# NikolaZubic/2dimageto3dmodel

Measured on NVIDIA H100. Metric: render+loss+GAN images/sec (cfg3: cfg2 render+loss at batch 32 + conv-GAN 256x256 G/D iteration, 1 G : 2 D, Adam), higher is better.
Workload: dtype tf32 (convs) / f32

## Files before the change

### 2dimageto3dmodel_b200/b3d/__init__.py

```python
import ctypes
import os

import torch

_HERE = os.path.dirname(os.path.abspath(__file__))
LIB_PATH = os.path.join(_HERE, "libb3d.so")

MODE_REFERENCE = 0
MODE_PAPER = 1
_MODES = {"R": MODE_REFERENCE, "reference": MODE_REFERENCE, "P": MODE_PAPER, "paper": MODE_PAPER,
          0: MODE_REFERENCE, 1: MODE_PAPER}


class B3DError(RuntimeError):
    pass


def _load():
    if not os.path.exists(LIB_PATH):
        raise B3DError(f"{LIB_PATH} is missing: build it with `make` (or __graft_entry__.build()). "
                       "There is no CPU fallback.")
    lib = ctypes.CDLL(LIB_PATH)
    lib.b3d_last_error.restype = ctypes.c_char_p
    lib.b3d_last_variant.restype = ctypes.c_char_p
# ... 6 lines not shown

_vp = ctypes.c_void_p
_i = ctypes.c_int
_f = ctypes.c_float
_sz = ctypes.c_size_t
_ll = ctypes.c_longlong


_signed = []


def _sig(name, *argtypes):
    fn = getattr(lib, name)
    fn.argtypes = list(argtypes)
    fn.restype = ctypes.c_int
    _signed.append(name)
    return fn


_sig("b3d_pc_bin_count", _i)
_sig("b3d_inception_input", _vp, _i, _i, _i, _i, _i, _i, _i, _vp, _vp)
_sig("b3d_maxpool3x3s2_nhwc", _vp, _i, _i, _i, _i, _vp, _i, _vp)
_sig("b3d_mean_hw_nhwc", _vp, _i, _i, _i, _vp, _vp)
_sig("b3d_fid_accumulate", _vp, _i, _i, _vp, _vp, _vp)
_sig("b3d_pc_project", _vp, _vp, _i, _i, _i, _f, _f, _vp, _vp, _vp, _vp, _vp, _vp, _vp)
_sig("b3d_pc_silhouette_fwd_hosttaps", _vp, _vp, _vp, _i, _vp, _i, _i, _i, _i, _vp, _vp, _sz, _vp)
_sig("b3d_pc_silhouette_bwd_hosttaps", _vp, _vp, _vp, _i, _vp, _vp, _i, _i, _i, _i, _vp, _vp, _vp, _sz, _vp)
_sig("b3d_pc_project_bwd", _vp, _vp, _vp, _vp, _i, _i, _i, _f, _f, _vp, _vp, _vp)
_sig("b3d_pc_splat_grid", _vp, _i, _i, _i, _i, _vp, _vp)
_sig("b3d_mesh_face_setup", _vp, _vp, _vp, _i, _vp, _i, _i, _i, _i, _vp, _vp, _vp, _vp)
_sig("b3d_mesh_render_fwd", _vp, _vp, _vp, _vp, _i, _i, _i, _i, _i, _i, _vp, _vp, _vp, _vp, _vp)
_sig("b3d_conv2d_tf32", _vp, _vp, _vp, _vp, _i, _i, _i, _i, _i, _i, _i, _i, _vp, _vp, _i, _i, _i, _i, _i, _i, _i, _i, _i,
     _f, _vp, _i, _vp, _i, _i, _vp, _vp)
_sig("b3d_conv2d_wgrad_tf32", _vp, _vp, _vp, _i, _i, _i, _i, _i, _i, _i, _i, _i, _i, _i, _i, _i, _i, _i, _vp)
_sig("b3d_conv2d_thin_fwd", _vp, _vp, _vp, _vp, _i, _i, _i, _i, _i, _i, _i, _i, _i, _i, _i, _i, _i, _f, _vp)
_sig("b3d_conv2d_thin_wgrad", _vp, _vp, _vp, _i, _i, _i, _i, _i, _i, _i, _i, _i, _i, _i, _i, _vp)
_sig("b3d_vertex_pipeline_fwd", _vp, _ll, _ll, _ll, _ll, _i, _i, _vp, _vp, _i, _i, _vp, _vp, _vp, _vp, _vp, _vp, _vp)
_sig("b3d_vertex_pipeline_bwd", _vp, _vp, _vp, _vp, _vp, _i, _i, _i, _i, _vp, _vp, _vp, _vp, _vp, _vp, _vp, _vp, _vp)
_sig("b3d_bank_forward", _vp, _vp, _i, _vp, _i, _vp, _i, _vp, _sz, _vp, _i, _vp)
_sig("b3d_bank_backward", _vp, _vp, _i, _vp, _i, _vp, _vp, _vp, _vp)
_sig("b3d_up2_fold", _vp, _vp, _i, _i, _vp)
_sig("b3d_pad_x_fwd", _vp, _vp, _ll, _i, _i, _i, _i, _vp)
_sig("b3d_pad_x_bwd", _vp, _vp, _ll, _i, _i, _i, _i, _vp)
_sig("b3d_stem_input_fwd", _vp, _vp, _vp, _i, _i, _i, _i, _i, _i, _i, _vp)
_sig("b3d_stem_input_bwd", _vp, _vp, _i, _i, _i, _i, _i, _i, _i, _vp)
_sig("b3d_leaky_bwd", _vp, _vp, _vp, _ll, _f, _vp)
_sig("b3d_fold_rows_fwd", _vp, _vp, _i, _i, _i, _i, _i, _i, _i, _vp)
_sig("b3d_fold_rows_bwd", _vp, _vp, _i, _i, _i, _i, _i, _i, _i, _vp)
_sig("b3d_wrap_x_inplace", _vp, _ll, _i, _i, _i, _i, _vp)
_sig("b3d_wrap_x_bwd_inplace", _vp, _ll, _i, _i, _i, _i, _vp)
_sig("b3d_pad_leaky_bias_bwd", _vp, _vp, _vp, _vp, _ll, _i, _i, _i, _i, _f, _vp)
_sig("b3d_vox_blur_axis", _vp, _vp, _vp, _i, _i, _i, _i, _i, _vp)
_sig("b3d_vox_scale_clamp", _vp, _vp, _vp, _i, _i, _vp)
_sig("b3d_vox_scale_clamp_bwd", _vp, _vp, _vp, _vp, _vp, _i, _i, _vp)
_sig("b3d_vox_termination", _vp, _i, _i, _i, _vp, _vp, _vp)
_sig("b3d_vox_termination_bwd", _vp, _vp, _i, _i, _i, _vp, _vp)
_sig("b3d_vox_splat_sorted", _vp, _vp, _i, _i, _i, _i, _vp, _vp)
_sig("b3d_vox_clamp01", _vp, ctypes.c_longlong, _vp)
_sig("b3d_vox_gather", _vp, _vp, _vp, _vp, _i, _i, _i, _i, _vp, _vp)
_sig("b3d_cbn_act_fwd", _vp, _vp, _vp, _vp, _i, _i, _vp, _i, _i, _i, _i, _i, _i, _i, _f, _i, _vp)
_sig("b3d_cbn_act_bwd1", _vp, _vp, _vp, _vp, _vp, _i, _i, _vp, _vp, _i, _vp, _vp, _i, _i, _vp, _vp, _i, _i, _i, _i, _i, _i, _i, _i,
     _f, _i, _vp)
_sig("b3d_cbn_act_bwd2", _vp, _vp, _vp, _vp, _vp, _i, _vp, _vp, _i, _f, _i, _i, _i, _i, _vp)
_sig("b3d_bn_sums", _vp, _ll, _i, _vp, _vp)
_sig("b3d_cbn_prepare", _vp, _i, _i, _i, _vp, ctypes.c_double, _f, _f, _i, _vp, _vp, _vp, _vp, _vp, _vp, _vp, _vp, _i, _i, _vp)
_sig("b3d_cbn_bwd_reduce", _vp, _vp, _i, _vp, _vp, _i, _i, _vp)
# ... 119 lines not shown
```

### 2dimageto3dmodel_b200/b3d/conv.py

```python
import ctypes

import torch

from . import B3DError, check, dev, last_variant, lib, ptr, stream_ptr
from .bank import LayerWeights

VARIANT_LOG = None


def _conv_call(fn, *args):
    rc = fn(*args)
    if VARIANT_LOG is not None and rc == 0:
        VARIANT_LOG.extend(v for v in last_variant().split(";") if v)
    return rc


def _ints(v):
    return (ctypes.c_int * len(v))(*v)


def _pad_last(t, mult):
    c = t.shape[-1]
    return t if c % mult == 0 else torch.nn.functional.pad(t, (0, mult - c % mult))


def taps_layout(weight):
    co, ci, kh, kw = weight.shape
    return weight.permute(2, 3, 0, 1).reshape(kh * kw, co, ci).contiguous()


def _d_layout(wf):
    return _pad_last(wf.transpose(1, 2), 32).contiguous()


def _thin(Cout, Cin, kh, kw, stride):
    return Cout <= 4 and Cin % 64 == 0 and kh == 5 and kw == 5 and stride == 1


class _ConvOpts(ctypes.Structure):
    _fields_ = [("mask", ctypes.c_void_p), ("mask_slope", ctypes.c_float), ("stats_sum_only", ctypes.c_int),
                ("x_row_pitch", ctypes.c_int), ("nclass", ctypes.c_int), ("class_ooy", ctypes.c_int * 4), ("class_oox", ctypes.c_int * 4)]


def _fprop(x, wt, bias, kh, kw, pad_y=0, stride=1, leaky=1.0, pad_out=0, pad_mode=1, x_crop=0, stats=None, fold_kh=0,
           fold_pad=0):
    N, H, W, _ = x.shape
    _, Cout, Cin = wt.shape
    if x_crop and stride != 1:
        raise B3DError("conv2d: x_crop needs stride 1")
    if pad_out and Cout % 4:
        raise B3DError("conv2d: pad_out needs Cout % 4 == 0")
    Hout = (H + 2 * fold_pad - fold_kh + 1) if fold_kh else (H + 2 * pad_y - kh) // stride + 1
    Wout = (W - 2 * x_crop - kw) // stride + 1
    OW = Wout + 2 * pad_out
    out = torch.empty(N, Hout, OW, Cout, device=x.device, dtype=torch.float32)
    optr = ctypes.c_void_p(out.data_ptr() + 4 * pad_out * Cout)
    b = dev(bias, "bias") if bias is not None else None
    st = stream_ptr(x)
    if _thin(Cout, Cin, kh, kw, stride):
        check(_conv_call(lib.b3d_conv2d_thin_fwd, ptr(x), ptr(wt), ptr(b), optr, N, H, W, Cin, Hout, Wout, Cout, kh, kw, pad_y,
                         x_crop, OW, Cout, float(leaky), st))
    else:
        if stats is not None and (bias is not None or leaky != 1.0 or stride != 1):
            raise B3DError("conv2d: output statistics are taken before bias / activation (plain stride-1 convs only)")
        dy = [r - pad_y for r in range(kh) for _ in range(kw)]
        dx = [s + x_crop for _ in range(kh) for s in range(kw)]
        check(_conv_call(lib.b3d_conv2d_tf32, ptr(x), ptr(wt), ptr(b), optr, N, H, W, Cin, Hout, Wout, Cout, kh * kw, _ints(dy),
                         _ints(dx), stride, stride, Hout, OW, Cout, 1, 1, 0, 0, float(leaky), None, 0, ptr(stats), fold_kh,
                         fold_pad, None, st))
    if pad_out:
        check(lib.b3d_wrap_x_inplace(ptr(out), N * Hout, Wout, Cout, pad_out, pad_mode, st))
    return out


def stride2_classes(kh, kw, pad_y, H, W):
    out = []
    for cy in range(2):
        for cx in range(2):
            rs = [(r, s) for r in range(kh) for s in range(kw) if (cy + pad_y - r) % 2 == 0 and (cx - s) % 2 == 0]
            out.append((cy, cx, rs, [(cy + pad_y - r) // 2 for r, s in rs], [(cx - s) // 2 for r, s in rs],
                        (H - cy + 1) // 2, (W - cx + 1) // 2))
    return out


def _merge_parity_classes(classes):
    return len(classes) == 4 and all(c[2] for c in classes) and len({(len(c[2]), c[5], c[6]) for c in classes}) == 1


def _dgrad(gy, wd, in_hw, kh, kw, pad_y=0, stride=1, x_crop=0, g_pitch=0, mask=None, slope=1.0, sums=None):
    gy = _pad_last(gy, 32)
    N, Hout, Wout, Cop = gy.shape
    Cin = wd.shape[1]
# ... 158 lines not shown
    x = xp_nchw.permute(0, 2, 3, 1)
    out = _UpConv.apply(x, lw.wf, lw_sc.wf if lw_sc is not None else None, lw, lw_sc, stats)
    y, sc = out if lw_sc is not None else (out, None)
    return y.permute(0, 3, 1, 2), sc.permute(0, 3, 1, 2) if sc is not None else None


def conv2d_nhwc(x, weight, bias=None, pad_y=0, stride=1, leaky=1.0, wt=None, pad_out=0, pad_mode=1, x_crop=0):
    x = dev(x, "x")
    Cout, Cin_w, kh, kw = weight.shape
    if Cin_w != x.shape[3]:
        raise B3DError(f"conv2d: input has {x.shape[3]} channels, weight expects {Cin_w}")
    wt = dev(wt if wt is not None else taps_layout(weight), "weight")
    return _fprop(x, wt, bias, kh, kw, pad_y, stride, leaky, pad_out, pad_mode, x_crop)


def conv2d_dgrad_nhwc(dy_, weight, in_hw, pad_y=0, stride=1, x_crop=0):
    Cout, Cin, kh, kw = weight.shape
    wd = _d_layout(weight.permute(2, 3, 0, 1).reshape(kh * kw, Cout, Cin))
    return _dgrad(dev(dy_, "grad_output"), wd, in_hw, kh, kw, pad_y, stride, x_crop)


def conv2d_wgrad_nhwc(dy_, x, kh, kw, pad_y=0, stride=1, x_crop=0):
    return _wgrad(dev(dy_, "grad_output"), dev(x, "input"), kh, kw, pad_y, stride, x_crop)


class ActLink:
    __slots__ = ("armed", "slope", "pad", "mode", "ptr", "shape", "want_gb", "gb", "done")

    def __init__(self):
        self.armed = self.done = False
        self.gb = None


class _Conv(torch.autograd.Function):
    @staticmethod
    def forward(ctx, x, w, bias, lw, pad_y, stride, leaky, pad_out, pad_mode, x_crop, stats=None, fold_raw=0, link_in=None,
                link_out=None, fold_fwd=False):
        x = dev(x.detach(), "x")
        if lw.wp is not None:
            raise B3DError("conv2d: a layer registered with up2 runs through conv2d_up2_banked")
        Cx = x.shape[3]
        fold_pad = 0
        if fold_raw:
            if not lw.fold or Cx != 8 or lw.Cin != 8 or stride != 1 or x_crop:
                raise B3DError("conv2d: on-the-fly fold needs a folded 8-channel stride-1 stem")
            fold_pad = pad_y
        elif Cx != lw.Cinp:
            if lw.fold or Cx != lw.Cin:
                raise B3DError(f"conv2d: input has {Cx} channels, the layer expects {lw.Cinp if lw.fold else lw.Cin}")
            x = _pad_last(x, 32)
        kh, kw = (1, lw.kw) if lw.fold else (lw.kh, lw.kw)
        if lw.fold:
            pad_y = 0
        wf, b = dev(lw.wf.detach(), "weight"), bias.detach() if bias is not None else None
        if fold_raw and fold_fwd:
            from .ew import fold_rows
            out = _fprop(fold_rows(x, lw.kh, fold_pad, lw.Cinp), wf, b, kh, kw, 0, stride, leaky, pad_out, pad_mode, x_crop, stats)
        else:
            out = _fprop(x, wf, b, kh, kw, pad_y, stride, leaky, pad_out, pad_mode, x_crop, stats, fold_raw, fold_pad)
        ctx.save_for_backward(x, out if (leaky != 1.0 or pad_out) else None)
        ctx.lw = lw
        ctx.cfg = (pad_y, stride, Cx, bias is not None, leaky, pad_out, pad_mode, x_crop, kh, kw, fold_raw, fold_pad)
        thin = _thin(lw.Cout, lw.Cinp, kh, kw, stride)
        ctx.link_in = link_in if (link_in is not None and link_in.armed and link_in.ptr == x.data_ptr() and link_in.shape == tuple(x.shape)
                                  and Cx == lw.Cinp and lw.Cinp % 32 == 0 and not fold_raw and not thin) else None
        ctx.link_out = None
        if link_out is not None and pad_out and leaky != 1.0 and lw.Cout % 32 == 0 and not thin:
            link_out.armed, link_out.slope, link_out.pad, link_out.mode = True, float(leaky), int(pad_out), int(pad_mode)
            link_out.ptr, link_out.shape, link_out.done = out.data_ptr(), tuple(out.shape), False
            link_out.want_gb = bias is not None and bool(ctx.needs_input_grad[2])
            ctx.link_out = link_out
        return out

    @staticmethod
    def backward(ctx, gy):
        x, y = ctx.saved_tensors
        lw = ctx.lw
        pad_y, stride, Cx, has_bias, leaky, pad_out, pad_mode, x_crop, kh, kw, fold_raw, fold_pad = ctx.cfg
        Cout, Cin = lw.Cout, lw.Cinp
        N, H, W, _ = x.shape
        gy = dev(gy, "grad_output")
        st = stream_ptr(gy)
        gb = None
        want_gb = has_bias and ctx.needs_input_grad[2]
        g_pitch = 0
        link_out = ctx.link_out
        if link_out is not None and link_out.done:
            link_out.done = False
# ... 10 lines not shown
            check(lib.b3d_pad_leaky_bias_bwd(ptr(gy), ptr(y), ptr(masked), ptr(gb), N * Ho, OW - 2 * pad_out, Cout, pad_out,
                                             pad_mode, float(leaky), st))
            gy = masked
        elif leaky != 1.0:
            masked = torch.empty_like(gy)
            check(lib.b3d_leaky_bwd(ptr(gy), ptr(y), ptr(masked), gy.numel(), float(leaky), st))
            gy = masked
        if gb is None and want_gb:
            gb = gy.sum(dim=(0, 1, 2))
        gx = gw = None
        if ctx.needs_input_grad[0]:
            link_in = ctx.link_in
            sums = torch.zeros(2 * Cin, device=gy.device, dtype=torch.float64) if link_in is not None and link_in.want_gb else None
            gx = _dgrad(gy, lw.wd if lw.wd is not None else _d_layout(lw.wf.detach()), (gy.shape[1] if fold_raw else H, W), kh,
                        kw, pad_y, stride, x_crop, g_pitch, x if link_in is not None else None,
                        link_in.slope if link_in is not None else 1.0, sums)
            if link_in is not None:
                check(lib.b3d_wrap_x_bwd_inplace(ptr(gx), N * H, W - 2 * link_in.pad, Cin, link_in.pad, link_in.mode, st))
                link_in.gb = sums[:Cin].float() if sums is not None else None
                link_in.done = True
            if fold_raw:
                graw = torch.empty(N, H, W, Cx, device=gy.device, dtype=torch.float32)
                check(lib.b3d_fold_rows_bwd(ptr(gx), ptr(graw), N, H, W, Cx, lw.kh, fold_pad, Cin, st))
                gx = graw
            elif Cx != Cin:
                gx = gx[..., :Cx]
        if ctx.needs_input_grad[1]:
            if fold_raw:
                gw = _wgrad(gy, x, kh, kw, fold_pad, stride, x_crop, lw.df, g_pitch, fold_raw, Cin)
            else:
                gw = _wgrad(gy, x, kh, kw, pad_y, stride, x_crop, lw.df, g_pitch)
            if lw.df is None:
                gw = gw[:, :lw.Cin]
        return gx, gw, gb, None, None, None, None, None, None, None, None, None, None, None, None


def fold_kh_weight(weight, cpad=0):
    Cout, Cin, kh, kw = weight.shape
    w = weight.permute(0, 2, 1, 3).reshape(Cout, kh * Cin, 1, kw)
    return torch.nn.functional.pad(w, (0, 0, 0, 0, 0, cpad)) if cpad else w


def conv2d(x_nchw, weight, bias=None, pad_y=0, stride=1, leaky=1.0, pad_out=0, pad_mode=1, x_crop=0):
    x = x_nchw.permute(0, 2, 3, 1)
    Cout, Cin, kh, kw = weight.shape
    if stride == 1 and kh > 1 and Cin * kh <= 64:
        from .ew import fold_rows
        cpad = (-kh * Cin) % 32
        x = fold_rows(x, kh, pad_y, kh * Cin + cpad)
        weight = fold_kh_weight(weight, cpad)
        Cout, Cin, kh, kw = weight.shape
        pad_y = 0
    lw = LayerWeights(dict(Cout=Cout, Cin=Cin, kh=kh, kw=kw, fold=0, Cinp=-(-Cin // 32) * 32, Coutp=-(-Cout // 32) * 32,
                           Tp=kh * kw))
    lw.wf = _pad_last(taps_layout(weight.detach()), 32)
    y = _Conv.apply(x, weight, bias, lw, int(pad_y), int(stride), float(leaky), int(pad_out), int(pad_mode), int(x_crop))
    return y.permute(0, 3, 1, 2)


def conv2d_banked(x_nchw, lw, pad_y=0, stride=1, leaky=1.0, pad_out=0, pad_mode=1, x_crop=0, stats=None, link_in=None, link_out=None):
    x = x_nchw.permute(0, 2, 3, 1)
    fold_raw, fold_fwd = 0, False
    if lw.fold:
        Wout = x.shape[2] - lw.kw + 1
        if (lw.Cin == 8 and lw.kw == 5 and lw.Cinp == 64 and stride == 1 and not x_crop and Wout % 128 == 0
                and x.shape[0] * x.shape[1] * (Wout // 128) >= 2 * torch.cuda.get_device_properties(x.device).multi_processor_count):
            fold_raw = lw.kh
            fold_fwd = torch.is_grad_enabled() and lw.wf.requires_grad
        else:
            from .ew import fold_rows
            x = fold_rows(x, lw.kh, pad_y, lw.Cinp)
    y = _Conv.apply(x, lw.wf, lw.bias, lw, int(pad_y), int(stride), float(leaky), int(pad_out), int(pad_mode), int(x_crop), stats,
                    fold_raw, link_in, link_out, fold_fwd)
    return y.permute(0, 3, 1, 2)
```

### 2dimageto3dmodel_b200/csrc/b3d_core.cu

```cuda
#include <atomic>
#include <stdarg.h>
#include <string.h>

#include "b3d_common.cuh"

namespace b3d {
static thread_local char g_err[512] = "";
static thread_local char g_variant[256] = "";
static std::atomic<uint64_t> g_launches{0};

void set_error(const char* fmt, ...) {
    va_list ap;
    va_start(ap, fmt);
    vsnprintf(g_err, sizeof(g_err), fmt, ap);
    va_end(ap);
}
void clear_variant() { g_variant[0] = 0; }
void add_variant(const char* fmt, ...) {
    size_t n = strlen(g_variant);
    if (n + 2 >= sizeof(g_variant)) return;
    if (n) g_variant[n++] = ';';
    va_list ap;
    va_start(ap, fmt);
    vsnprintf(g_variant + n, sizeof(g_variant) - n, fmt, ap);
    va_end(ap);
}
void count_launch(int n) { g_launches.fetch_add((uint64_t)n, std::memory_order_relaxed); }
}

extern "C" {
const char* b3d_last_error(void) { return b3d::g_err; }
const char* b3d_last_variant(void) { return b3d::g_variant; }
int b3d_version(void) { return 440; }
uint64_t b3d_launch_count(void) { return b3d::g_launches.load(std::memory_order_relaxed); }
}
```

### 2dimageto3dmodel_b200/csrc/tc_conv.cu

```cuda
#include "tc_common.cuh"

namespace {

constexpr int BM = 128;
constexpr int BK = 32;
constexpr int MMA_K = 8;
constexpr int MAX_TAPS = 25;
constexpr int NTHREADS = 384;

struct ConvParams {
    int N, Hout, Wout, Cout;
    int BW, BH, BI;
    int tiles_x, tiles_y;
    int xbase;
    int ntaps, kslices;
    int sy, sx;
    int dy[MAX_TAPS], dx[MAX_TAPS];
    int wtap[MAX_TAPS];
    int OH, OW, OC, osy, osx;
    float leaky;
    double* stats;
    int fold;
    int fold_y0;
    int mask;
// ... 19 lines not shown

__device__ __forceinline__ uint32_t mask_offset(int px, int ch) { return px * 128 + ((((ch >> 2) ^ px) & 7) << 4) + (ch & 3) * 4; }

template <int BN>
constexpr bool kCoop = BN > 128;
template <int BN>
constexpr int kBlocks = (kCoop<BN> ? BN / 2 : BN) / 64;
template <int BN>
constexpr int kEmptyArrivals = kCoop<BN> ? 8 : 4;
template <int BN>
constexpr int kLeaderArrivals = kEmptyArrivals<BN> / (kCoop<BN> ? 2 : 1);
static_assert(kLeaderArrivals<64> == 4 && kLeaderArrivals<128> == 4 && kLeaderArrivals<256> == 4,
              "a leader stands for the 4 warps of its warpgroup");
template <int BN>
constexpr int kMaskGroup = kCoop<BN> ? 4 : 2;
__host__ __device__ constexpr int mask_chunk_channel(int i, int G) { return 128 * ((i % G) / 2) + 64 * (i / G) + 32 * (i % 2); }

template <int BN, int STAGES, int KW, bool FOLD>
__device__ __forceinline__ void mainloop(float (&acc)[kBlocks<BN>][BM / 2], unsigned char* base, uint64_t* full, uint64_t* empty,
                                         int KI, uint32_t& git, uint32_t& phase, int cb, bool leader, const int* shift) {
    constexpr int A_BYTES = CSmem<BN, STAGES, KW>::A_BYTES, STAGE = CSmem<BN, STAGES, KW>::STAGE_BYTES;
    for (int it = 0; it < KI; ++it, ++git) {
        const int s = git % STAGES;
        tc::mbar_wait(full + s, (phase >> s) & 1);
        phase ^= 1u << s;
        const uint32_t a = tc::smem_u32(base + s * STAGE), b = a + A_BYTES + cb * 128;
        tc::wgmma_fence();
#pragma unroll
        for (int t = 0; t < KW; ++t) {
            const uint32_t shifted = a + (KW > 1 ? shift[t] * 128 : 0);
#pragma unroll
            for (int k = 0; k < BK / MMA_K; ++k) {
                const uint32_t acc_flag = (it | t | k) ? 1u : 0u;
                const uint64_t dp = FOLD ? tc::desc_k32(a + k * (BM * 32)) : tc::desc_k128(shifted + k * MMA_K * 4);
#pragma unroll
                for (int m = 0; m < kBlocks<BN>; ++m)
                    tc::Wgmma<BM>::mma(acc[m], tc::desc_k128(b + t * (BN * 128) + m * (64 * 128) + k * MMA_K * 4), dp, acc_flag);
            }
        }
        tc::wgmma_commit();
        tc::wgmma_wait<1>();
        if (it > 0 && leader) tc::mbar_arrive(empty + (git - 1) % STAGES, kLeaderArrivals<BN>);
    }
    tc::wgmma_wait<0>();
    if (KI > 0 && leader) tc::mbar_arrive(empty + (git - 1) % STAGES, kLeaderArrivals<BN>);
}

struct TileAt {
    int n0, y0, x0;
    size_t base;
    int lbw, lbwh;
};
__device__ __forceinline__ void tile_origin(const ConvParams& p, TileAt& t, int tile, int cls) {
    t.x0 = p.xbase + (tile % p.tiles_x) * p.BW;
    t.y0 = (tile / p.tiles_x) % p.tiles_y * p.BH;
    t.n0 = tile / (p.tiles_x * p.tiles_y) * p.BI;
    t.base = (((size_t)t.n0 * p.OH + (size_t)(p.osy * t.y0 + p.cooy[cls])) * p.OW + (size_t)(p.osx * t.x0 + p.coox[cls])) * p.OC;
}
__device__ __forceinline__ bool tile_pixel(const ConvParams& p, const TileAt& t, int px, uint32_t& rel) {
    const int bi = px >> t.lbwh, by = (px >> t.lbw) & (p.BH - 1), bx = px & (p.BW - 1);
    rel = bi * p.esn + by * p.esy + bx * p.esx;
    return t.n0 + bi < p.N && t.y0 + by < p.Hout && t.x0 + bx < p.Wout;
}

template <int G, int STAGES>
__device__ __forceinline__ void mask_bits(uint32_t (&neg)[2], uint32_t mstage, int cw, int lane, uint64_t* empty, uint32_t g0) {
    int q;
// ... 37 lines not shown
        for (int e1 = 0; e1 < 2; ++e1) {
            uint32_t rel;
            const bool valid = tile_pixel(p, t, 8 * j + q + e1, rel);
#pragma unroll
            for (int e2 = 0; e2 < 2; ++e2) {
                float v = acc[4 * j + 2 * e2 + e1];
                if constexpr (MASKED) v *= (neg[j / 8] >> (4 * (j % 8) + 2 * e2 + e1)) & 1u ? p.mslope : 1.f;
                v = valid ? v : 0.f;
                sum[e2] += v;
                sq[e2] += v * v;
                if (valid && cok[e2]) {
                    const float o = v + bv[e2];
                    out0[rel + 8 * e2] = o >= 0.f ? o : o * p.leaky;
                }
            }
        }
    }
    if (p.stats) {
#pragma unroll
        for (int e = 0; e < 2; ++e) {
            sum[e] += __shfl_xor_sync(0xffffffffu, sum[e], 1);
            sum[e] += __shfl_xor_sync(0xffffffffu, sum[e], 2);
            sq[e] += __shfl_xor_sync(0xffffffffu, sq[e], 1);
            sq[e] += __shfl_xor_sync(0xffffffffu, sq[e], 2);
            if ((lane & 3) == 0 && cok[e]) {
                atomicAdd(p.stats + c0 + cw + 8 * e, (double)sum[e]);
                if (!p.stats_sum) atomicAdd(p.stats + p.Cout + c0 + cw + 8 * e, (double)sq[e]);
            }
        }
    }
}

constexpr int PRODUCER_REGS = 24, CONSUMER_REGS = 240;

template <int BN, int STAGES, int KW>
__global__ void __launch_bounds__(NTHREADS, 1)
conv_wgmma_kernel(const __grid_constant__ CUtensorMap tmap_x, const __grid_constant__ CUtensorMap tmap_w,
                  const __grid_constant__ CUtensorMap tmap_m, const ConvParams p, const float* __restrict__ bias,
                  float* __restrict__ out, int tiles, int work_items) {
    using S = CSmem<BN, STAGES, KW>;
    constexpr bool COOP = kCoop<BN>;
    constexpr int OWNERS = COOP ? 1 : 2;
    constexpr int G = kMaskGroup<BN>;
    static_assert(G <= STAGES, "the mask stages of one block do not fit the ring");
    extern __shared__ unsigned char smem_raw[];
    unsigned char* base = reinterpret_cast<unsigned char*>((reinterpret_cast<uintptr_t>(smem_raw) + 1023) & ~uintptr_t(1023));
    uint64_t* full = reinterpret_cast<uint64_t*>(base + STAGES * S::STAGE_BYTES);
    uint64_t* empty = full + OWNERS * STAGES;
    static_assert((OWNERS + 1) * STAGES * 8 <= 256, "barriers do not fit their area");
    if (threadIdx.x == 0) {
        tc::tma_prefetch_desc(&tmap_x);
        tc::tma_prefetch_desc(&tmap_w);
        if (p.mask) tc::tma_prefetch_desc(&tmap_m);
        for (int s = 0; s < STAGES; ++s) {
            for (int o = 0; o < OWNERS; ++o) tc::mbar_init(full + o * STAGES + s, 1);
            tc::mbar_init(empty + s, kEmptyArrivals<BN>);
        }
        tc::fence_barrier_init();
    }
    __syncthreads();
    const int KI = p.ntaps / KW * p.kslices;
    const int MS = p.mask ? BN / 32 : 0;
    const int wg = threadIdx.x >> 7;

    if (wg == 0) {
        tc::setmaxnreg_dec<PRODUCER_REGS>();
        if (threadIdx.x == 0) {
            uint32_t git = 0;
            for (int w = blockIdx.x, k = 0; w < work_items; w += gridDim.x, ++k) {
                uint64_t* fb = full + (COOP ? 0 : (k & 1) * STAGES);
                const int cls = w % p.ncls, wq = w / p.ncls, tb = cls * p.ntaps;
                int t = wq % tiles;
                const int c0 = (wq / tiles) * BN;
                const int x0 = p.xbase + (t % p.tiles_x) * p.BW;
                t /= p.tiles_x;
                const int y0 = (t % p.tiles_y) * p.BH, n0 = (t / p.tiles_y) * p.BI;
                for (int it = 0; it < KI; ++it, ++git) {
                    const int s = git % STAGES;
                    tc::mbar_wait(empty + s, ((git / STAGES) & 1) ^ 1);
                    const int tap = it / p.kslices * KW, ks = it % p.kslices;
                    unsigned char* a = base + s * S::STAGE_BYTES;
                    tc::mbar_arrive_expect_tx(fb + s, S::TX_BYTES);
                    if (KW > 1)
                        tc::tma_load_4d(a, &tmap_x, fb + s, ks * BK, x0 + p.dx0, y0 + p.dy[tb + tap], n0);
                    else if (p.fold)
                        tc::tma_load_4d(a, &tmap_x, fb + s, 0, x0 + p.dx[tb + tap], y0 + p.fold_y0 + 4 * ks, n0);
                    else
                        tc::tma_load_4d(a, &tmap_x, fb + s, ks * BK, p.sx * x0 + p.dx[tb + tap], p.sy * y0 + p.dy[tb + tap], n0);
                    tc::tma_load_3d(a + S::A_BYTES, &tmap_w, fb + s, ks * BK, c0, p.wtap[tb + tap]);
                }
                const int mx = p.osx * x0 + p.coox[cls], my = p.osy * y0 + p.cooy[cls];
                for (int m = 0; m < MS; ++m, ++git) {
                    const int s = git % STAGES;
                    tc::mbar_wait(empty + s, ((git / STAGES) & 1) ^ 1);
                    tc::mbar_arrive_expect_tx(fb + s, MASK_BYTES);
                    tc::tma_load_4d(base + s * S::STAGE_BYTES, &tmap_m, fb + s, c0 + mask_chunk_channel(m, G), mx, my, n0);
                }
            }
        }
        return;
    }
    tc::setmaxnreg_inc<CONSUMER_REGS>();

    const int h = wg - 1, tid = threadIdx.x & 127, lane = tid & 31;
    float acc[kBlocks<BN>][BM / 2];
#pragma unroll
    for (int m = 0; m < kBlocks<BN>; ++m)
#pragma unroll
        for (int i = 0; i < BM / 2; ++i) acc[m][i] = 0.f;
    uint32_t git = 0, phase = 0;
    const uint32_t ring = tc::smem_u32(base);
    TileAt at;
    at.lbw = __ffs(p.BW) - 1;
    at.lbwh = at.lbw + __ffs(p.BH) - 1;
    uint64_t* fb = full + (COOP ? 0 : h * STAGES);
    const int cb = COOP ? 128 * h : 0;
    const int cw = (tid >> 5) * 16 + (lane >> 2);
    const int mine = (COOP ? 2 * h : 0) + (tid >> 6);
    for (int k = COOP ? 0 : h;; k += COOP ? 1 : 2) {
        const int w = blockIdx.x + k * gridDim.x;
        if (w >= work_items) break;
        git = (uint32_t)k * (KI + MS);
        const int wq = w / p.ncls, tile = wq % tiles, c0 = (wq / tiles) * BN + cb;
        tile_origin(p, at, tile, w % p.ncls);
        if (KW == 1 && p.fold) mainloop<BN, STAGES, KW, true>(acc, base, fb, empty, KI, git, phase, cb, tid == 0, p.shift);
        else mainloop<BN, STAGES, KW, false>(acc, base, fb, empty, KI, git, phase, cb, tid == 0, p.shift);
        uint32_t neg[kBlocks<BN>][2] = {};
        if (p.mask) {
#pragma unroll
            for (int m = 0; m < kBlocks<BN>; ++m, git += G) {
                uint32_t mstage = 0;
#pragma unroll
                for (int i = 0; i < G; ++i) {
                    const int s = (git + i) % STAGES;
                    tc::mbar_wait(fb + s, (phase >> s) & 1);
                    phase ^= 1u << s;
                    if (i == mine) mstage = ring + s * S::STAGE_BYTES;
                }
                mask_bits<G, STAGES>(neg[m], mstage, cw, lane, empty, git);
            }
        }
#pragma unroll
        for (int m = 0; m < kBlocks<BN>; ++m) {
            if (p.mask) epilogue_block<true>(acc[m], neg[m], p, at, bias, out, c0 + 64 * m, cw, lane);
            else epilogue_block<false>(acc[m], neg[m], p, at, bias, out, c0 + 64 * m, cw, lane);
        }
    }
}

struct WgradParams {
    int N, Hout, Wout, Cout, Cin;
    int BWk, BHk;
    int kx, ky;
    int kh, kw, pad_y, st;
    int xoff;
    int splits;
    int tapmajor;
    int tstep;
// ... 371 lines not shown
    }
    return best;
}

template <int BN, int STAGES, int KW = 1>
int launch_conv(const CUtensorMap& mx, const CUtensorMap& mw, const CUtensorMap& mm, const ConvParams& p, const float* bias, float* out,
                int tiles, cudaStream_t st) {
    using S = CSmem<BN, STAGES, KW>;
    static_assert(S::TOTAL <= 227 * 1024, "conv pipeline does not fit shared memory");
    B3D_CUDA_OK(cudaFuncSetAttribute(conv_wgmma_kernel<BN, STAGES, KW>, cudaFuncAttributeMaxDynamicSharedMemorySize, S::TOTAL));
    const int work = tiles * b3d::ceil_div(p.Cout, BN) * p.ncls;
    const int sms = tc::num_sms();
    conv_wgmma_kernel<BN, STAGES, KW><<<work < sms ? work : sms, NTHREADS, S::TOTAL, st>>>(mx, mw, mm, p, bias, out, tiles, work);
    B3D_LAUNCH_OK();
    if (KW > 1) b3d::add_variant("conv_wgmma_rowwin<%d,%d,%d>", BN, KW, STAGES);
    else b3d::add_variant("conv_wgmma<%d,%d>", BN, STAGES);
    return B3D_OK;
}

template <int BN>
int launch_rowwin(int kw, const CUtensorMap& mx, const CUtensorMap& mw, const CUtensorMap& mm, const ConvParams& p, const float* bias,
                  float* out, int tiles, cudaStream_t st) {
    if (kw == 2) return launch_conv<BN, BN == 64 ? 5 : 4, 2>(mx, mw, mm, p, bias, out, tiles, st);
    if (kw == 3) return launch_conv<BN, BN == 64 ? 4 : 3, 3>(mx, mw, mm, p, bias, out, tiles, st);
    return launch_conv<BN, BN == 64 ? 3 : 2, 5>(mx, mw, mm, p, bias, out, tiles, st);
}

int pow2_floor(int v) {
    int p = 1;
    while (p * 2 <= v) p *= 2;
    return p;
}

}

extern "C" {

int b3d_conv2d_tf32(const float* x, const float* wt, const float* bias, float* out, int N, int H, int W, int Cin,
                    int Hout, int Wout, int Cout, int ntaps, const int* dy, const int* dx, int sy, int sx, int OH,
                    int OW, int OC, int osy, int osx, int ooy, int oox, float leaky, const int* wtap,
                    int wtaps_total, double* stats, int fold_kh, int fold_pad, const b3d_conv_opts* opts, void* stream) {
    B3D_REQUIRE(N > 0 && H > 0 && W > 0 && Hout > 0 && Wout > 0 && Cout > 0, B3D_EINVAL, "b3d_conv2d_tf32: bad sizes");
    B3D_REQUIRE(Cin > 0 && Cin % BK == 0, B3D_EINVAL, "b3d_conv2d_tf32: Cin=%d must be a multiple of %d", Cin, BK);
    B3D_REQUIRE(ntaps >= 1 && ntaps <= MAX_TAPS && dy && dx, B3D_EINVAL, "b3d_conv2d_tf32: bad taps");
    B3D_REQUIRE(x && wt && out, B3D_EINVAL, "b3d_conv2d_tf32: null pointer");
    B3D_REQUIRE(sy >= 1 && sy <= 2 && sx >= 1 && sx <= 2, B3D_EINVAL, "b3d_conv2d_tf32: stride must be 1 or 2");
    if (!wtap) wtaps_total = ntaps;
    B3D_REQUIRE(wtaps_total >= ntaps || wtap, B3D_EINVAL, "b3d_conv2d_tf32: bad weight tap count");
    for (int t = 0; wtap && t < ntaps; ++t)
        B3D_REQUIRE(wtap[t] >= 0 && wtap[t] < wtaps_total, B3D_EINVAL, "b3d_conv2d_tf32: weight tap %d out of range", wtap[t]);
    B3D_CHECK_ALIGNED(x);
    B3D_CHECK_ALIGNED(wt);
    b3d::clear_variant();

    const float* mask = opts ? opts->mask : nullptr;
    const float mslope = opts ? opts->mask_slope : 1.f;
    B3D_REQUIRE(!mask || (reinterpret_cast<uintptr_t>(mask) % 16 == 0 && OC % 4 == 0), B3D_EINVAL,
                "b3d_conv2d_tf32: the mask needs a 16-byte aligned base and OC %% 4 == 0 (OC=%d)", OC);
    const int stats_sum = (opts && opts->stats_sum_only) ? 1 : 0;
    const int xpitch = (opts && opts->x_row_pitch) ? opts->x_row_pitch : W;
    const int ncls = (opts && opts->nclass > 1) ? opts->nclass : 1;
    B3D_REQUIRE(ncls <= 4 && ntaps % ncls == 0 && (ncls == 1 || (sy == 1 && sx == 1 && fold_kh == 0)), B3D_EINVAL,
                "b3d_conv2d_tf32: nclass=%d needs <= 4 equal tap groups of a stride-1 launch", ncls);
    const int tpc = ntaps / ncls;
    int cooy[4] = {ooy, ooy, ooy, ooy}, coox[4] = {oox, oox, oox, oox};
    for (int c = 0; c < ncls && ncls > 1; ++c) { cooy[c] = opts->class_ooy[c]; coox[c] = opts->class_oox[c]; }
    B3D_REQUIRE(xpitch >= W && (fold_kh == 0 || xpitch == W), B3D_EINVAL, "b3d_conv2d_tf32: x_row_pitch=%d must be >= W=%d (and absent with the on-the-fly fold)", xpitch, W);
    if (fold_kh > 0) {
        B3D_REQUIRE(fold_kh <= 8 && Cin == 32 * ((8 * fold_kh + 31) / 32) && sy == 1 && sx == 1 && !wtap && Wout % BM == 0,
                    B3D_EINVAL, "b3d_conv2d_tf32: on-the-fly fold needs 8 input channels, stride 1 and Wout %% 128 == 0 (Wout=%d)", Wout);
    }
    bool tiles = ncls == 4 && osy == 2 && osx == 2 && OH == 2 * Hout && OW == 2 * Wout;
    for (int c = 0, seen = 0; tiles && c < 4; ++c) {
        const int bit = 1 << (2 * cooy[c] + coox[c]);
// ... 33 lines not shown
        const int wspan = xhi - xlo;
        ConvParams p{};
        p.N = N; p.Hout = Hout; p.Wout = xhi; p.Cout = Cout; p.xbase = xlo;
        p.BW = pow2_floor(wspan < BM ? wspan : BM);
        p.BH = pow2_floor(Hout < BM / p.BW ? Hout : BM / p.BW);
        p.BI = BM / (p.BW * p.BH);
        p.tiles_x = b3d::ceil_div(wspan, p.BW);
        p.tiles_y = b3d::ceil_div(Hout, p.BH);
        const int tiles = p.tiles_x * p.tiles_y * b3d::ceil_div(N, p.BI);
        p.ntaps = tpc; p.kslices = Cin / BK; p.sy = sy; p.sx = sx; p.ncls = ncls;
        for (int t = 0; t < ntaps; ++t) { p.dy[t] = dy[t]; p.dx[t] = dx[t]; p.wtap[t] = wtap ? wtap[t] : t; }
        for (int c = 0; c < 4; ++c) { p.cooy[c] = cooy[c]; p.coox[c] = coox[c]; }
        p.OH = OH; p.OW = OW; p.OC = OC; p.osy = osy; p.osx = osx;
        p.leaky = leaky;
        p.stats = stats;
        p.mask = mask != nullptr; p.mslope = mslope; p.stats_sum = stats_sum;
        p.fold = fold_kh; p.fold_y0 = -fold_pad;
        {
            const unsigned long long esn = p.BI > 1 ? (unsigned long long)OH * OW * OC : 0, esy = p.BH > 1 ? (unsigned long long)osy * OW * OC : 0,
                                     esx = (unsigned long long)osx * OC;
            B3D_REQUIRE((p.BI - 1) * esn + (p.BH - 1) * esy + (p.BW - 1) * esx + OC < (1ull << 32), B3D_EINVAL,
                        "b3d_conv2d_tf32: a %d x %d x %d pixel tile spans more than 2^32 elements of the output", p.BI, p.BH, p.BW);
            p.esn = (uint32_t)esn; p.esy = (uint32_t)esy; p.esx = (uint32_t)esx;
        }
        CUtensorMap mm{};
        if (mask) {
            const uint64_t dims[4] = {(uint64_t)OC, (uint64_t)OW, (uint64_t)OH, (uint64_t)N};
            const uint64_t strides[3] = {(uint64_t)OC * 4, (uint64_t)OW * OC * 4, (uint64_t)OH * OW * OC * 4};
            const uint32_t box[4] = {(uint32_t)BK, (uint32_t)(osx * (p.BW - 1) + 1), (uint32_t)(osy * (p.BH - 1) + 1), (uint32_t)p.BI};
            const uint32_t es[4] = {1, (uint32_t)osx, (uint32_t)osy, 1};
            if (int rc = tc::make_tmap_f32(&mm, mask, 4, dims, strides, box, es)) return rc;
        }
        CUtensorMap mx;
        if (g_kw && wspan >= BM) {
            p.dx0 = g_step > 0 ? dx[0] : dx[g_kw - 1];
            for (int t = 0; t < g_kw; ++t) p.shift[t] = dx[t] - p.dx0;
            const uint64_t dims[4] = {(uint64_t)Cin, (uint64_t)W, (uint64_t)H, (uint64_t)N};
            const uint64_t strides[3] = {(uint64_t)Cin * 4, (uint64_t)xpitch * Cin * 4, (uint64_t)H * xpitch * Cin * 4};
            const uint32_t box[4] = {(uint32_t)BK, (uint32_t)(BM + g_kw - 1), 1, 1};
            if (int rc = tc::make_tmap_f32(&mx, x, 4, dims, strides, box)) return rc;
            CUtensorMap mwr;
            const uint64_t wdims[3] = {(uint64_t)Cin, (uint64_t)Cout, (uint64_t)wtaps_total};
            const uint64_t wstrides[2] = {(uint64_t)Cin * 4, (uint64_t)Cout * Cin * 4};
            const uint32_t wbox[3] = {(uint32_t)BK, (uint32_t)BN, (uint32_t)((g_kw - 1) * g_wstep + 1)};
            const uint32_t wes[3] = {1, 1, (uint32_t)g_wstep};
            if (int rc = tc::make_tmap_f32(&mwr, wt, 3, wdims, wstrides, wbox, wes)) return rc;
            return BN == 128 ? launch_rowwin<128>(g_kw, mx, mwr, mm, p, bias, out, tiles, st)
                             : launch_rowwin<64>(g_kw, mx, mwr, mm, p, bias, out, tiles, st);
        }
        if (fold_kh > 0) {
            B3D_REQUIRE(p.BH == 1 && p.BI == 1, B3D_EINVAL, "b3d_conv2d_tf32: on-the-fly fold needs one-row tiles");
            const uint64_t dims[4] = {8, (uint64_t)W, (uint64_t)H, (uint64_t)N};
            const uint64_t strides[3] = {32, (uint64_t)W * 32, (uint64_t)H * W * 32};
            const uint32_t box[4] = {8, (uint32_t)p.BW, 4, 1};
            if (int rc = tc::make_tmap_f32(&mx, x, 4, dims, strides, box, nullptr, CU_TENSOR_MAP_SWIZZLE_32B)) return rc;
        } else {
            const uint64_t dims[4] = {(uint64_t)Cin, (uint64_t)W, (uint64_t)H, (uint64_t)N};
            const uint64_t strides[3] = {(uint64_t)Cin * 4, (uint64_t)xpitch * Cin * 4, (uint64_t)H * xpitch * Cin * 4};
            const uint32_t box[4] = {(uint32_t)BK, (uint32_t)(sx * (p.BW - 1) + 1), (uint32_t)(sy * (p.BH - 1) + 1), (uint32_t)p.BI};
            const uint32_t es[4] = {1, (uint32_t)sx, (uint32_t)sy, 1};
            if (int rc = tc::make_tmap_f32(&mx, x, 4, dims, strides, box, es)) return rc;
        }
        if (BN == 256) return launch_conv<256, 4>(mx, mw, mm, p, bias, out, tiles, st);
        if (BN == 128) return launch_conv<128, 6>(mx, mw, mm, p, bias, out, tiles, st);
        return launch_conv<64, 8>(mx, mw, mm, p, bias, out, tiles, st);
    };
    const int bw_full = pow2_floor(Wout < BM ? Wout : BM);
    const int rem = Wout % bw_full;
    if (rem != 0 && rem * 8 <= bw_full && Wout > bw_full) {
        const int rc = run(0, Wout - rem);
        return rc ? rc : run(Wout - rem, Wout);
    }
    return run(0, Wout);
}

int b3d_conv2d_wgrad_tf32(const float* dy, const float* x, float* dw, int N, int H, int W, int Cin, int Hout, int Wout,
                          int Cout, int kh, int kw, int pad_y, int stride, int x_off, int tap_major, int fold_kh, int dy_row_pitch,
                          void* stream) {
    B3D_REQUIRE(N > 0 && Cin > 0 && Cout > 0 && H > 0 && W > 0 && Hout > 0 && Wout > 0, B3D_EINVAL,
                "b3d_conv2d_wgrad_tf32: bad sizes");
    B3D_REQUIRE(kh * kw <= MAX_TAPS && (stride == 1 || stride == 2) && x_off > -kw, B3D_EINVAL, "b3d_conv2d_wgrad_tf32: bad kernel/stride");
    B3D_REQUIRE(dy && x && dw, B3D_EINVAL, "b3d_conv2d_wgrad_tf32: null pointer");
    B3D_REQUIRE(Cin % 32 == 0 && Cout % 32 == 0, B3D_EINVAL,
                "b3d_conv2d_wgrad_tf32: Cin=%d and Cout=%d must be multiples of 32 (pad the channels with zeros)", Cin, Cout);
    B3D_CHECK_ALIGNED(dy);
    B3D_CHECK_ALIGNED(x);
    b3d::clear_variant();
    if (tap_major) B3D_CHECK_ALIGNED(dw);
    WgradParams p{};
    p.N = N; p.Hout = Hout; p.Wout = Wout; p.Cout = Cout; p.Cin = Cin;
    const uint64_t dpitch = dy_row_pitch > 0 ? dy_row_pitch : Wout;
    B3D_REQUIRE(dpitch >= (uint64_t)Wout, B3D_EINVAL, "b3d_conv2d_wgrad_tf32: dy_row_pitch=%d must be >= Wout=%d", dy_row_pitch, Wout);
    cudaStream_t st = (cudaStream_t)stream;
    if (fold_kh > 0) {
        B3D_REQUIRE(fold_kh > 4 && fold_kh <= 8 && Cin == 64 && kh == 1 && kw == STEM_KW && stride == 1 && x_off == 0 &&
                        Cout % 64 == 0 && W == Wout + STEM_KW - 1 && Hout == H + 2 * pad_y - fold_kh + 1,
                    B3D_EINVAL, "b3d_conv2d_wgrad_tf32: the raw-input stem weight gradient needs 4 < fold_kh <= 8 rows folded into "
                    "64 channels, a 1x5 stride-1 filter, Cout %% 64 == 0 and the x padding in the input");
        p.BWk = BK; p.BHk = 1;
        p.kx = b3d::ceil_div(Wout, BK);
        p.ky = Hout;
        p.kh = 1; p.kw = kw; p.pad_y = pad_y; p.st = 1; p.tapmajor = tap_major ? 1 : 0;
        p.splits = wgrad_splits(Cout / 64, (long long)N * p.kx * p.ky);
        CUtensorMap mdy, mx;
        {
            const uint64_t dims[5] = {32, (uint64_t)Wout, (uint64_t)Hout, (uint64_t)N, (uint64_t)Cout / 32};
// ... 57 lines not shown
```

### include/b3d.h

```cpp
#ifndef B3D_H_
#define B3D_H_

#include <stddef.h>
#include <stdint.h>

#ifdef __cplusplus
extern "C" {
#endif

#if defined(__GNUC__)
#define B3D_API __attribute__((visibility("default")))
#else
#define B3D_API
#endif

#define B3D_OK 0
#define B3D_EINVAL (-1)
#define B3D_EALIGN (-2)
#define B3D_ECUDA (-3)

#define B3D_MODE_REFERENCE 0
#define B3D_MODE_PAPER 1

B3D_API const char* b3d_last_error(void);
// ... 85 lines not shown
                              void* stream);
B3D_API int b3d_flat_loss_bwd(const float* norms, const int32_t* ff, int B, int F, int K,
                              const float* gloss, float* dnorms, void* stream);

B3D_API int b3d_rgba_mse_iou_fwd(const float* image, const float* alpha, const float* target, int B, int H,
                                 int W, float* loss, int32_t* counts, void* stream);
B3D_API int b3d_rgba_mse_bwd(const float* image, const float* alpha, const float* target, int B, int H,
                             int W, const float* gloss, float* d_image, float* d_alpha, void* stream);

B3D_API int b3d_rgba_l1_iou_fwd(const float* image, const float* alpha, const float* target, int B, int H,
                                int W, float* loss, int32_t* counts, void* stream);
B3D_API int b3d_rgba_l1_bwd(const float* image, const float* alpha, const float* target, int B, int H,
                            int W, const float* gloss, float* d_image, float* d_alpha, void* stream);

B3D_API int b3d_chamfer_nn(const float* query, const float* cand, int B, int N, int M, float* dist,
                           int32_t* idx, void* stream);
B3D_API int b3d_chamfer_bwd(const float* query, const float* cand, const int32_t* idx, const float* gdist,
                            int B, int N, int M, float* dquery, float* dcand, void* stream);

typedef struct b3d_conv_opts {
    const float* mask;
    float mask_slope;
    int stats_sum_only;
    int x_row_pitch;
    int nclass;
    int class_ooy[4];
    int class_oox[4];
} b3d_conv_opts;
B3D_API int b3d_conv2d_tf32(const float* x, const float* wt, const float* bias, float* out, int N, int H, int W,
                            int Cin, int Hout, int Wout, int Cout, int ntaps, const int* dy, const int* dx,
                            int sy, int sx, int OH, int OW, int OC, int osy, int osx, int ooy, int oox,
                            float leaky, const int* wtap, int wtaps_total, double* stats, int fold_kh,
                            int fold_pad, const b3d_conv_opts* opts, void* stream);

B3D_API int b3d_conv2d_wgrad_tf32(const float* dy, const float* x, float* dw, int N, int H, int W, int Cin,
                                  int Hout, int Wout, int Cout, int kh, int kw, int pad_y, int stride,
                                  int x_off, int tap_major, int fold_kh, int dy_row_pitch, void* stream);

B3D_API int b3d_conv2d_thin_fwd(const float* x, const float* wt, const float* bias, float* out, int N, int H, int W, int Cin,
                                int Hout, int Wout, int Cout, int kh, int kw, int pad_y, int x_off, int OW, int OC,
                                float leaky, void* stream);
B3D_API int b3d_conv2d_thin_wgrad(const float* dy, const float* x, float* dw, int N, int H, int W, int Cin, int Hout,
                                  int Wout, int Cout, int kh, int kw, int pad_y, int x_off, int tap_major, void* stream);

B3D_API int b3d_vertex_record_bytes(void);
B3D_API int b3d_vertex_pipeline_fwd(const float* dmap, long long sn, long long sc, long long sy, long long sx, int h, int w,
                                    const void* rec, const void* sgn, int B, int V, const float* scale, const float* trans,
                                    const float* rot, const float* z0, float* raw, float* vtx, void* stream);
B3D_API int b3d_vertex_pipeline_bwd(const float* g_raw, const float* g_vtx, const float* raw, const void* rec, const void* sgn,
                                    int B, int V, int h, int w, const float* scale, const float* trans, const float* rot,
                                    const float* z0, float* d_dmap, float* d_scale, float* d_trans, float* d_z0, void* stream);

B3D_API int b3d_bank_layer_bytes(void);
B3D_API int b3d_bank_forward(const void* layers, const void* items_wtu, int n_wtu, const void* items_wv, int n_wv,
                             const void* items_emit, int n_emit, float* scratch, size_t scratch_bytes, float* out,
                             int training, void* stream);
B3D_API int b3d_bank_backward(const void* layers, const void* items_dot, int n_dot, const void* items_emit, int n_emit,
                              float* out, const float* df, float* dw, void* stream);
B3D_API int b3d_up2_fold(const float* dpt, float* df, int Cout, int Cin, void* stream);

B3D_API int b3d_pad_x_fwd(const float* x, float* out, long long rows, int W, int C, int amount, int mode, void* stream);
B3D_API int b3d_pad_x_bwd(const float* gout, float* gx, long long rows, int W, int C, int amount, int mode, void* stream);
B3D_API int b3d_stem_input_fwd(const float* x, const float* pos, float* out, int N, int C1, int C2, int H, int W, int amount,
                               int mode, void* stream);
B3D_API int b3d_stem_input_bwd(const float* gout, float* gx, int N, int C1, int C2, int H, int W, int amount, int mode,
                               void* stream);
// ... 81 lines not shown
```

Measured before the change: 1599.

## Add row-window stem conv that folds kernel rows on the fly for 1x5 filters

Adds a new stem forward path for the 8-channel, 5-wide folded stem conv. A TMA box spanning BM+4 columns and 4 rows is loaded once per k-slice, and the five horizontal taps are taken as shifted descriptors into that window. This avoids materialising the fold_rows tensor and re-loading the input per tap. It is enabled only for large outputs (at least 2^21 pixels), and the FOLD mainloop template is widened to KW=5 with BN=64.

```diff
diff --git a/2dimageto3dmodel_b200/b3d/__init__.py b/2dimageto3dmodel_b200/b3d/__init__.py
--- a/2dimageto3dmodel_b200/b3d/__init__.py
+++ b/2dimageto3dmodel_b200/b3d/__init__.py
@@ -62,6 +62,7 @@
 _sig("b3d_mesh_render_fwd", _vp, _vp, _vp, _vp, _i, _i, _i, _i, _i, _i, _vp, _vp, _vp, _vp, _vp)
 _sig("b3d_conv2d_tf32", _vp, _vp, _vp, _vp, _i, _i, _i, _i, _i, _i, _i, _i, _vp, _vp, _i, _i, _i, _i, _i, _i, _i, _i, _i,
      _f, _vp, _i, _vp, _i, _i, _vp, _vp)
+_sig("b3d_conv2d_stem_tf32", _vp, _vp, _vp, _vp, _i, _i, _i, _i, _i, _i, _i, _vp, _i, _i, _i, _f, _i, _i, _vp)
 _sig("b3d_conv2d_wgrad_tf32", _vp, _vp, _vp, _i, _i, _i, _i, _i, _i, _i, _i, _i, _i, _i, _i, _i, _i, _i, _vp)
 _sig("b3d_conv2d_thin_fwd", _vp, _vp, _vp, _vp, _i, _i, _i, _i, _i, _i, _i, _i, _i, _i, _i, _i, _i, _f, _vp)
 _sig("b3d_conv2d_thin_wgrad", _vp, _vp, _vp, _i, _i, _i, _i, _i, _i, _i, _i, _i, _i, _i, _i, _vp)
diff --git a/2dimageto3dmodel_b200/b3d/conv.py b/2dimageto3dmodel_b200/b3d/conv.py
--- a/2dimageto3dmodel_b200/b3d/conv.py
+++ b/2dimageto3dmodel_b200/b3d/conv.py
@@ -43,7 +43,7 @@
 
 
 def _fprop(x, wt, bias, kh, kw, pad_y=0, stride=1, leaky=1.0, pad_out=0, pad_mode=1, x_crop=0, stats=None, fold_kh=0,
-           fold_pad=0):
+           fold_pad=0, fold_win=False):
     N, H, W, _ = x.shape
     _, Cout, Cin = wt.shape
     if x_crop and stride != 1:
@@ -57,7 +57,12 @@
     optr = ctypes.c_void_p(out.data_ptr() + 4 * pad_out * Cout)
     b = dev(bias, "bias") if bias is not None else None
     st = stream_ptr(x)
-    if _thin(Cout, Cin, kh, kw, stride):
+    if fold_win:
+        if not fold_kh or stats is not None or kh != 1 or kw != 5 or stride != 1 or x_crop:
+            raise B3DError("conv2d: the row-window stem forward needs the on-the-fly fold of a 1 x 5 folded filter")
+        check(_conv_call(lib.b3d_conv2d_stem_tf32, ptr(x), ptr(wt), ptr(b), optr, N, H, W, Cin, Hout, Wout, Cout, _ints(list(range(kw))),
+                         Hout, OW, Cout, float(leaky), fold_kh, fold_pad, st))
+    elif _thin(Cout, Cin, kh, kw, stride):
         check(_conv_call(lib.b3d_conv2d_thin_fwd, ptr(x), ptr(wt), ptr(b), optr, N, H, W, Cin, Hout, Wout, Cout, kh, kw, pad_y,
                          x_crop, OW, Cout, float(leaky), st))
     else:
@@ -282,10 +287,13 @@
         self.gb = None
 
 
+STEM_WINDOW_MIN_PIXELS = 1 << 21
+
+
 class _Conv(torch.autograd.Function):
     @staticmethod
     def forward(ctx, x, w, bias, lw, pad_y, stride, leaky, pad_out, pad_mode, x_crop, stats=None, fold_raw=0, link_in=None,
-                link_out=None, fold_fwd=False):
+                link_out=None, fold_fwd=False, fold_win=False):
         x = dev(x.detach(), "x")
         if lw.wp is not None:
             raise B3DError("conv2d: a layer registered with up2 runs through conv2d_up2_banked")
@@ -303,7 +311,9 @@
         if lw.fold:
             pad_y = 0
         wf, b = dev(lw.wf.detach(), "weight"), bias.detach() if bias is not None else None
-        if fold_raw and fold_fwd:
+        if fold_raw and fold_win:
+            out = _fprop(x, wf, b, kh, kw, pad_y, stride, leaky, pad_out, pad_mode, x_crop, stats, fold_raw, fold_pad, True)
+        elif fold_raw and fold_fwd:
             from .ew import fold_rows
             out = _fprop(fold_rows(x, lw.kh, fold_pad, lw.Cinp), wf, b, kh, kw, 0, stride, leaky, pad_out, pad_mode, x_crop, stats)
         else:
@@ -380,7 +390,7 @@
                 gw = _wgrad(gy, x, kh, kw, pad_y, stride, x_crop, lw.df, g_pitch)
             if lw.df is None:
                 gw = gw[:, :lw.Cin]
-        return gx, gw, gb, None, None, None, None, None, None, None, None, None, None, None, None
+        return gx, gw, gb, None, None, None, None, None, None, None, None, None, None, None, None, None
 
 
 def fold_kh_weight(weight, cpad=0):
@@ -408,16 +418,17 @@
 
 def conv2d_banked(x_nchw, lw, pad_y=0, stride=1, leaky=1.0, pad_out=0, pad_mode=1, x_crop=0, stats=None, link_in=None, link_out=None):
     x = x_nchw.permute(0, 2, 3, 1)
-    fold_raw, fold_fwd = 0, False
+    fold_raw, fold_fwd, fold_win = 0, False, False
     if lw.fold:
         Wout = x.shape[2] - lw.kw + 1
         if (lw.Cin == 8 and lw.kw == 5 and lw.Cinp == 64 and stride == 1 and not x_crop and Wout % 128 == 0
                 and x.shape[0] * x.shape[1] * (Wout // 128) >= 2 * torch.cuda.get_device_properties(x.device).multi_processor_count):
             fold_raw = lw.kh
-            fold_fwd = torch.is_grad_enabled() and lw.wf.requires_grad
+            fold_win = x.shape[0] * (x.shape[1] + 2 * pad_y - lw.kh + 1) * Wout >= STEM_WINDOW_MIN_PIXELS
+            fold_fwd = not fold_win and torch.is_grad_enabled() and lw.wf.requires_grad
         else:
             from .ew import fold_rows
             x = fold_rows(x, lw.kh, pad_y, lw.Cinp)
     y = _Conv.apply(x, lw.wf, lw.bias, lw, int(pad_y), int(stride), float(leaky), int(pad_out), int(pad_mode), int(x_crop), stats,
-                    fold_raw, link_in, link_out, fold_fwd)
+                    fold_raw, link_in, link_out, fold_fwd, fold_win)
     return y.permute(0, 3, 1, 2)
diff --git a/2dimageto3dmodel_b200/csrc/b3d_core.cu b/2dimageto3dmodel_b200/csrc/b3d_core.cu
--- a/2dimageto3dmodel_b200/csrc/b3d_core.cu
+++ b/2dimageto3dmodel_b200/csrc/b3d_core.cu
@@ -31,6 +31,6 @@
 extern "C" {
 const char* b3d_last_error(void) { return b3d::g_err; }
 const char* b3d_last_variant(void) { return b3d::g_variant; }
-int b3d_version(void) { return 440; }
+int b3d_version(void) { return 450; }
 uint64_t b3d_launch_count(void) { return b3d::g_launches.load(std::memory_order_relaxed); }
 }
diff --git a/2dimageto3dmodel_b200/csrc/tc_conv.cu b/2dimageto3dmodel_b200/csrc/tc_conv.cu
--- a/2dimageto3dmodel_b200/csrc/tc_conv.cu
+++ b/2dimageto3dmodel_b200/csrc/tc_conv.cu
@@ -75,7 +75,8 @@
 #pragma unroll
             for (int k = 0; k < BK / MMA_K; ++k) {
                 const uint32_t acc_flag = (it | t | k) ? 1u : 0u;
-                const uint64_t dp = FOLD ? tc::desc_k32(a + k * (BM * 32)) : tc::desc_k128(shifted + k * MMA_K * 4);
+                const uint64_t dp = FOLD ? tc::desc_k32(a + k * ((BM + KW - 1) * 32) + (KW > 1 ? shift[t] * 32 : 0))
+                                         : tc::desc_k128(shifted + k * MMA_K * 4);
 #pragma unroll
                 for (int m = 0; m < kBlocks<BN>; ++m)
                     tc::Wgmma<BM>::mma(acc[m], tc::desc_k128(b + t * (BN * 128) + m * (64 * 128) + k * MMA_K * 4), dp, acc_flag);
@@ -179,6 +180,9 @@
 }
 
 constexpr int PRODUCER_REGS = 24, CONSUMER_REGS = 240;
+
+template <int BN, int KW>
+constexpr bool kFoldable = KW == 1 || (KW == 5 && BN == 64);
 
 template <int BN, int STAGES, int KW>
 __global__ void __launch_bounds__(NTHREADS, 1)
@@ -228,7 +232,9 @@
                     const int tap = it / p.kslices * KW, ks = it % p.kslices;
                     unsigned char* a = base + s * S::STAGE_BYTES;
                     tc::mbar_arrive_expect_tx(fb + s, S::TX_BYTES);
-                    if (KW > 1)
+                    if (KW > 1 && p.fold)
+                        tc::tma_load_4d(a, &tmap_x, fb + s, 0, x0 + p.dx0, y0 + p.fold_y0 + 4 * ks, n0);
+                    else if (KW > 1)
                         tc::tma_load_4d(a, &tmap_x, fb + s, ks * BK, x0 + p.dx0, y0 + p.dy[tb + tap], n0);
                     else if (p.fold)
                         tc::tma_load_4d(a, &tmap_x, fb + s, 0, x0 + p.dx[tb + tap], y0 + p.fold_y0 + 4 * ks, n0);
@@ -270,7 +276,7 @@
         git = (uint32_t)k * (KI + MS);
         const int wq = w / p.ncls, tile = wq % tiles, c0 = (wq / tiles) * BN + cb;
         tile_origin(p, at, tile, w % p.ncls);
-        if (KW == 1 && p.fold) mainloop<BN, STAGES, KW, true>(acc, base, fb, empty, KI, git, phase, cb, tid == 0, p.shift);
+        if (kFoldable<BN, KW> && p.fold) mainloop<BN, STAGES, KW, kFoldable<BN, KW>>(acc, base, fb, empty, KI, git, phase, cb, tid == 0, p.shift);
         else mainloop<BN, STAGES, KW, false>(acc, base, fb, empty, KI, git, phase, cb, tid == 0, p.shift);
         uint32_t neg[kBlocks<BN>][2] = {};
         if (p.mask) {
@@ -708,14 +714,10 @@
     return p;
 }
 
-}
-
-extern "C" {
-
-int b3d_conv2d_tf32(const float* x, const float* wt, const float* bias, float* out, int N, int H, int W, int Cin,
-                    int Hout, int Wout, int Cout, int ntaps, const int* dy, const int* dx, int sy, int sx, int OH,
-                    int OW, int OC, int osy, int osx, int ooy, int oox, float leaky, const int* wtap,
-                    int wtaps_total, double* stats, int fold_kh, int fold_pad, const b3d_conv_opts* opts, void* stream) {
+int conv2d_tf32(const float* x, const float* wt, const float* bias, float* out, int N, int H, int W, int Cin, int Hout, int Wout,
+                int Cout, int ntaps, const int* dy, const int* dx, int sy, int sx, int OH, int OW, int OC, int osy, int osx, int ooy,
+                int oox, float leaky, const int* wtap, int wtaps_total, double* stats, int fold_kh, int fold_pad,
+                const b3d_conv_opts* opts, bool fold_win, void* stream) {
     B3D_REQUIRE(N > 0 && H > 0 && W > 0 && Hout > 0 && Wout > 0 && Cout > 0, B3D_EINVAL, "b3d_conv2d_tf32: bad sizes");
     B3D_REQUIRE(Cin > 0 && Cin % BK == 0, B3D_EINVAL, "b3d_conv2d_tf32: Cin=%d must be a multiple of %d", Cin, BK);
     B3D_REQUIRE(ntaps >= 1 && ntaps <= MAX_TAPS && dy && dx, B3D_EINVAL, "b3d_conv2d_tf32: bad taps");
@@ -815,6 +817,23 @@
             if (int rc = tc::make_tmap_f32(&mm, mask, 4, dims, strides, box, es)) return rc;
         }
         CUtensorMap mx;
+        if (fold_win) {
+            bool taps_ok = ntaps == 5 && BN == 64 && p.BW == BM && p.BH == 1 && p.BI == 1;
+            for (int t = 1; taps_ok && t < 5; ++t) taps_ok = dx[t] == dx[0] + t;
+            B3D_REQUIRE(taps_ok, B3D_EINVAL, "b3d_conv2d_stem_tf32: needs five horizontally consecutive taps, Cout <= 64 and Wout %% %d == 0", BM);
+            p.dx0 = dx[0];
+            for (int t = 0; t < 5; ++t) p.shift[t] = dx[t] - dx[0];
+            const uint64_t dims[4] = {8, (uint64_t)W, (uint64_t)H, (uint64_t)N};
+            const uint64_t strides[3] = {32, (uint64_t)W * 32, (uint64_t)H * W * 32};
+            const uint32_t box[4] = {8, (uint32_t)(BM + 4), 4, 1};
+            if (int rc = tc::make_tmap_f32(&mx, x, 4, dims, strides, box, nullptr, CU_TENSOR_MAP_SWIZZLE_32B)) return rc;
+            CUtensorMap mwr;
+            const uint64_t wdims[3] = {(uint64_t)Cin, (uint64_t)Cout, (uint64_t)wtaps_total};
+            const uint64_t wstrides[2] = {(uint64_t)Cin * 4, (uint64_t)Cout * Cin * 4};
+            const uint32_t wbox[3] = {(uint32_t)BK, (uint32_t)BN, 5};
+            if (int rc = tc::make_tmap_f32(&mwr, wt, 3, wdims, wstrides, wbox)) return rc;
+            return launch_rowwin<64>(5, mx, mwr, mm, p, bias, out, tiles, st);
+        }
         if (g_kw && wspan >= BM) {
             p.dx0 = g_step > 0 ? dx[0] : dx[g_kw - 1];
             for (int t = 0; t < g_kw; ++t) p.shift[t] = dx[t] - p.dx0;
@@ -855,6 +874,27 @@
         return rc ? rc : run(Wout - rem, Wout);
     }
     return run(0, Wout);
+}
+
+}
+
+extern "C" {
+
+int b3d_conv2d_tf32(const float* x, const float* wt, const float* bias, float* out, int N, int H, int W, int Cin,
+                    int Hout, int Wout, int Cout, int ntaps, const int* dy, const int* dx, int sy, int sx, int OH,
+                    int OW, int OC, int osy, int osx, int ooy, int oox, float leaky, const int* wtap,
+                    int wtaps_total, double* stats, int fold_kh, int fold_pad, const b3d_conv_opts* opts, void* stream) {
+    return conv2d_tf32(x, wt, bias, out, N, H, W, Cin, Hout, Wout, Cout, ntaps, dy, dx, sy, sx, OH, OW, OC, osy, osx, ooy, oox, leaky,
+                       wtap, wtaps_total, stats, fold_kh, fold_pad, opts, false, stream);
+}
+
+int b3d_conv2d_stem_tf32(const float* x, const float* wt, const float* bias, float* out, int N, int H, int W, int Cin, int Hout,
+                         int Wout, int Cout, const int* dx, int OH, int OW, int OC, float leaky, int fold_kh, int fold_pad,
+                         void* stream) {
+    B3D_REQUIRE(fold_kh > 0 && dx, B3D_EINVAL, "b3d_conv2d_stem_tf32: needs fold_kh > 0 and the five taps' x offsets");
+    const int dy[5] = {0, 0, 0, 0, 0};
+    return conv2d_tf32(x, wt, bias, out, N, H, W, Cin, Hout, Wout, Cout, 5, dy, dx, 1, 1, OH, OW, OC, 1, 1, 0, 0, leaky, nullptr, 5,
+                       nullptr, fold_kh, fold_pad, nullptr, true, stream);
 }
 
 int b3d_conv2d_wgrad_tf32(const float* dy, const float* x, float* dw, int N, int H, int W, int Cin, int Hout, int Wout,
diff --git a/include/b3d.h b/include/b3d.h
--- a/include/b3d.h
+++ b/include/b3d.h
@@ -141,6 +141,9 @@
                             int sy, int sx, int OH, int OW, int OC, int osy, int osx, int ooy, int oox,
                             float leaky, const int* wtap, int wtaps_total, double* stats, int fold_kh,
                             int fold_pad, const b3d_conv_opts* opts, void* stream);
+B3D_API int b3d_conv2d_stem_tf32(const float* x, const float* wt, const float* bias, float* out, int N, int H, int W, int Cin,
+                                 int Hout, int Wout, int Cout, const int* dx, int OH, int OW, int OC, float leaky, int fold_kh,
+                                 int fold_pad, void* stream);
 
 B3D_API int b3d_conv2d_wgrad_tf32(const float* dy, const float* x, float* dw, int N, int H, int W, int Cin,
                                   int Hout, int Wout, int Cout, int kh, int kw, int pad_y, int stride,
```

Measured after the change: 1628, median of 6. +1.8%, better.
